# toutane/arcanefem

Hardware: AMD Instinct MI355X
Metric: MDoF/s assembly + CG iter/s, Poisson-3D P1 at 1/2/4/8 MI355X (higher is better)
Workload: dtype f64; 1 GPU; C2 Poisson-3D P1; n=215, dof_total=10077696, nnz_rank0=150048286, parallelism=z-slab x1, RCCL halo + all-reduce in CG

## Files before the change

arcanefem_amd/_capi.py:

```python
from __future__ import annotations

import ctypes
import os

_HERE = os.path.dirname(os.path.abspath(__file__))
LIB_PATH = os.environ.get("AFEM_LIB") or os.path.join(_HERE, "libafem.so")

AFEM_OK = 0
AFEM_MEM_HOST = 0
AFEM_MEM_DEVICE = 1
AFEM_RHS_ADD = 0
AFEM_RHS_SET = 1
AFEM_SOLVER_AUTO = 0
AFEM_SOLVER_PCG = 1
AFEM_SOLVER_DIRECT = 2
AFEM_NEUMANN_VALUE = 0
AFEM_NEUMANN_NORMAL = 1
AFEM_NEUMANN_TRACTION = 2
UNIQUE_ID_BYTES = 128
ERRORS = {1: "ArgumentException", 2: "HipError", 3: "NotImplementedException", 4: "StateError",
          5: "NotFound", 6: "CommError", 7: "LimitExceeded"}


class AfemError(RuntimeError):
# ... 2 lines not shown
        super().__init__(f"{func}: [{ERRORS.get(code, code)}] {msg}")


class MeshInfo(ctypes.Structure):
    _fields_ = [("dim", ctypes.c_int32), ("nb_node_per_cell", ctypes.c_int32), ("n_nodes", ctypes.c_int64),
                ("n_own_nodes", ctypes.c_int64), ("n_cells", ctypes.c_int64)]


class SubdomainInfo(ctypes.Structure):
    _fields_ = [("n_own_nodes", ctypes.c_int64), ("n_nodes", ctypes.c_int64), ("n_cells", ctypes.c_int64),
                ("n_neighbors", ctypes.c_int), ("n_send", ctypes.c_int64), ("n_recv", ctypes.c_int64)]


class CsrView(ctypes.Structure):
    _fields_ = [("n_block_rows", ctypes.c_int64), ("n_block_cols", ctypes.c_int64), ("nnz_blocks", ctypes.c_int64),
                ("block_size", ctypes.c_int32), ("ordered_per_block", ctypes.c_int32), ("rows", ctypes.c_void_p),
                ("columns", ctypes.c_void_p), ("values", ctypes.c_void_p)]


class AssemblyView(ctypes.Structure):
    _fields_ = [("n_rows", ctypes.c_int64), ("n_nodes", ctypes.c_int64), ("n_cells", ctypes.c_int64),
                ("nb_node_per_cell", ctypes.c_int32), ("block_size", ctypes.c_int32),
                ("ordered_per_block", ctypes.c_int32), ("dim", ctypes.c_int32), ("cell_node", ctypes.c_void_p),
                ("coords", ctypes.c_void_p), ("rows", ctypes.c_void_p), ("columns", ctypes.c_void_p),
                ("values", ctypes.c_void_p), ("error_flag", ctypes.c_void_p), ("stream", ctypes.c_void_p)]


class FunctorPlan(ctypes.Structure):
    _fields_ = [("n_units", ctypes.c_int64), ("n_stages", ctypes.c_int64), ("n_entries", ctypes.c_int64),
                ("rows_per_layer", ctypes.c_int32), ("width", ctypes.c_int32), ("nbuf", ctypes.c_int32),
                ("wide", ctypes.c_int32), ("block_size", ctypes.c_int32), ("nb_node_per_cell", ctypes.c_int32),
                ("ordered_per_block", ctypes.c_int32), ("lattice", ctypes.c_int32), ("units", ctypes.c_void_p),
                ("stage_ptr", ctypes.c_void_p), ("layer_rows", ctypes.c_void_p), ("entries", ctypes.c_void_p),
                ("entries2", ctypes.c_void_p), ("rows", ctypes.c_void_p), ("values", ctypes.c_void_p),
                ("stream", ctypes.c_void_p), ("patterns", ctypes.c_void_p), ("n_patterns", ctypes.c_int64),
                ("packed", ctypes.c_int32), ("reserved0", ctypes.c_int32)]


class Csr32View(ctypes.Structure):
    _fields_ = [("n_rows", ctypes.c_int64), ("nnz", ctypes.c_int64), ("rows", ctypes.c_void_p),
                ("rows_nb_column", ctypes.c_void_p), ("columns", ctypes.c_void_p), ("values", ctypes.c_void_p),
                ("identity", ctypes.c_int32)]


class BsrStats(ctypes.Structure):
    _fields_ = [("n_incidences", ctypes.c_int64), ("inc_table_entries", ctypes.c_int64),
                ("max_row_len", ctypes.c_int32), ("rows_per_block", ctypes.c_int32), ("max_seg", ctypes.c_int64),
                ("max_slice_nodes", ctypes.c_int32), ("max_slice_width", ctypes.c_int32),
                ("n_slices", ctypes.c_int64), ("brick_order", ctypes.c_int32), ("uniform_slices", ctypes.c_int32),
                ("last_kernel", ctypes.c_int32), ("stencil_slices", ctypes.c_int32),
                ("stencil_sig", ctypes.c_int32), ("shared_strip_slices", ctypes.c_int64),
                ("uniform_instance_slices", ctypes.c_int64), ("general_slices", ctypes.c_int64),
                ("cube_lattice", ctypes.c_int32), ("cube_axes", ctypes.c_int32),
                ("cube_row_stride", ctypes.c_int64)]


class SolverOpts(ctypes.Structure):
    _fields_ = [("method", ctypes.c_int32), ("max_iter", ctypes.c_int32), ("rtol", ctypes.c_double),
                ("atol", ctypes.c_double), ("check_every", ctypes.c_int32), ("fixed_iterations", ctypes.c_int32),
                ("initial_guess", ctypes.c_int32), ("precond_block", ctypes.c_int32), ("multigrid", ctypes.c_int32),
                ("profile_comm", ctypes.c_int32), ("amg", ctypes.c_int32)]


class SolveStats(ctypes.Structure):
    _fields_ = [("iterations", ctypes.c_int32), ("converged", ctypes.c_int32), ("rel_residual", ctypes.c_double),
                ("residual_norm", ctypes.c_double), ("solve_ms", ctypes.c_double), ("spmv_kernel", ctypes.c_int32),
                ("halo_wait_ms", ctypes.c_double), ("allreduce_ms", ctypes.c_double), ("halo_bytes", ctypes.c_int64),
                ("n_halo", ctypes.c_int32), ("n_allreduce", ctypes.c_int32), ("amg_levels", ctypes.c_int32),
                ("amg_coarse_rows", ctypes.c_int64), ("amg_complexity", ctypes.c_double),
                ("amg_setup_ms", ctypes.c_double), ("precond_ms", ctypes.c_double)]


class StepTiming(ctypes.Structure):
    _fields_ = [("assemble_ms", ctypes.c_double), ("rhs_ms", ctypes.c_double), ("bc_ms", ctypes.c_double),
                ("solve_ms", ctypes.c_double), ("precond_ms", ctypes.c_double), ("update_ms", ctypes.c_double),
                ("total_ms", ctypes.c_double), ("iterations", ctypes.c_int32), ("reserved0", ctypes.c_int32),
                ("nnz_blocks", ctypes.c_int64), ("n_incidences", ctypes.c_int64), ("n_nodes", ctypes.c_int64),
                ("n_own_nodes", ctypes.c_int64)]


ALLREDUCE_FN = ctypes.CFUNCTYPE(ctypes.c_int, ctypes.c_void_p, ctypes.POINTER(ctypes.c_double), ctypes.c_int64)
EXCHANGE_FN = ctypes.CFUNCTYPE(ctypes.c_int, ctypes.c_void_p, ctypes.c_int, ctypes.POINTER(ctypes.c_int32),
                               ctypes.POINTER(ctypes.c_double), ctypes.POINTER(ctypes.c_int64),
                               ctypes.POINTER(ctypes.c_double), ctypes.POINTER(ctypes.c_int64))


class HostTransport(ctypes.Structure):
    _fields_ = [("user", ctypes.c_void_p), ("allreduce_sum", ALLREDUCE_FN), ("exchange", EXCHANGE_FN)]


class NewmarkParams(ctypes.Structure):
    _fields_ = [("E", ctypes.c_double), ("nu", ctypes.c_double), ("rho", ctypes.c_double), ("dt", ctypes.c_double),
                ("body_force", ctypes.c_double * 3), ("penalty", ctypes.c_double), ("gamma", ctypes.c_double),
                ("beta", ctypes.c_double), ("etam", ctypes.c_double), ("etak", ctypes.c_double),
                ("alpm", ctypes.c_double), ("alpf", ctypes.c_double), ("scheme", ctypes.c_int32),
                ("reserved0", ctypes.c_int32)]


P = ctypes.c_void_p
PP = ctypes.POINTER(ctypes.c_void_p)
I32 = ctypes.c_int32
I64 = ctypes.c_int64
U64 = ctypes.c_uint64
D = ctypes.c_double
INT = ctypes.c_int

SIGNATURES = {
# ... 124 lines not shown
```

arcanefem_amd/core.py:

```python
from __future__ import annotations

import ctypes

import numpy as np

from . import _capi as C
from ._capi import AfemError, call

__all__ = ["AfemError", "Context", "Mesh", "BSRFormat", "DoFLinearSystem", "HipDoFLinearSystemFactory",
           "applyNeumannToRhs", "device_count", "set_variant", "structured_halo_plan"]


def _ptr(a: np.ndarray):
    return ctypes.c_void_p(a.ctypes.data)


def _rhs_mode(mode: str) -> int:
    if mode not in ("add", "set"):
        raise ValueError(f"rhs_mode must be 'add' or 'set', got {mode!r}")
    return C.AFEM_RHS_ADD if mode == "add" else C.AFEM_RHS_SET


NEUMANN_MODES = {"value": C.AFEM_NEUMANN_VALUE, "normal": C.AFEM_NEUMANN_NORMAL, "traction": C.AFEM_NEUMANN_TRACTION}

# ... 175 lines not shown
    def __init__(self, mesh: Mesh, nb_dof: int = 1):
        self.mesh = mesh
        self.nb_dof = nb_dof
        self.h = None

    def initialize(self, use_csr_in_linear_system: bool = True):
        h = ctypes.c_void_p()
        call("afem_bsr_create", self.mesh.h, self.nb_dof, 1 if use_csr_in_linear_system else 0, ctypes.byref(h))
        self.h = h
        return self

    def computeSparsity(self):
        call("afem_bsr_compute_sparsity", self.h)

    def assemblePoissonP1(self, coef: float = 1.0, f: float | None = None, rhs_dptr: int | None = None,
                          rhs_mode: str = "add"):
        call("afem_bsr_assemble_poisson_p1_ex", self.h, coef, 0.0 if f is None else f,
             ctypes.c_void_p(rhs_dptr) if rhs_dptr else None, _rhs_mode(rhs_mode))

    def assembleElasticityP1(self, lam: float, mu2: float):
        call("afem_bsr_assemble_elasticity_p1", self.h, lam, mu2)

    def assembleElasticityP1Ex(self, lam: float, mu2: float, mass_coef: float = 0.0, body_force=None,
                               rhs_dptr: int | None = None, rhs_mode: str = "add"):
        f = None
        if body_force is not None:
            f = (ctypes.c_double * 3)(*[float(x) for x in body_force])
        call("afem_bsr_assemble_elasticity_p1_ex", self.h, lam, mu2, mass_coef, f,
             ctypes.c_void_p(rhs_dptr) if rhs_dptr else None, _rhs_mode(rhs_mode))

    def resetMatrixValues(self):
        call("afem_bsr_reset_values", self.h)

    def setValue(self, row: int, col: int, v: float):
        call("afem_bsr_set_value", self.h, row, col, v)

    def getValue(self, row: int, col: int) -> float:
        v = ctypes.c_double()
        call("afem_bsr_get_value", self.h, row, col, ctypes.byref(v))
        return v.value

    def toLinearSystem(self, ls: "DoFLinearSystem"):
        call("afem_bsr_to_linear_system", self.h, ls.impl)

    def view(self) -> C.CsrView:
        v = C.CsrView()
        call("afem_bsr_view", self.h, ctypes.byref(v))
        return v

    def stats(self) -> dict:
        s = C.BsrStats()
        call("afem_bsr_get_stats", self.h, ctypes.byref(s))
        return {k: getattr(s, k) for k, _ in s._fields_}

    def functor_plan(self) -> dict:
        p = C.FunctorPlan()
        call("afem_bsr_functor_plan", self.h, ctypes.byref(p))
        return {k: getattr(p, k) for k, _ in p._fields_ if not k in
                ("units", "stage_ptr", "layer_rows", "entries", "entries2", "rows", "values", "stream",
                 "patterns", "reserved0")}

    def download(self):
        v = self.view()
        rows = np.empty(v.n_block_rows + 1, dtype=np.int64)
        cols = np.empty(v.nnz_blocks, dtype=np.int32)
        vals = np.empty(v.nnz_blocks * v.block_size ** 2, dtype=np.float64)
        call("afem_bsr_download", self.h, _ptr(rows), _ptr(cols), _ptr(vals))
        return rows, cols, vals

    def export_csr32(self):
        n = ctypes.c_int64()
        nnz = ctypes.c_int64()
        call("afem_bsr_get_sizes", self.h, ctypes.byref(n), ctypes.byref(nnz))
        rows = np.empty(n.value, dtype=np.int32)
        rnc = np.empty(n.value, dtype=np.int32)
        cols = np.empty(nnz.value, dtype=np.int32)
        vals = np.empty(nnz.value, dtype=np.float64)
        call("afem_bsr_export_csr32", self.h, _ptr(rows), _ptr(rnc), _ptr(cols), _ptr(vals))
        return rows, rnc, cols, vals

    def close(self):
        if self.h:
            call("afem_bsr_destroy", self.h)
            self.h = None


class DoFLinearSystem:

    def __init__(self):
        self.impl = None
        self.ctx = None
        self.factory = None
        self.n_rows = 0
        self.n_cols = 0

    def setLinearSystemFactory(self, factory: "HipDoFLinearSystemFactory"):
        self.factory = factory

    def initialize(self, ctx: Context, n_rows: int, n_cols_local: int | None = None, solver_name: str = "Solver"):
        factory = self.factory or HipDoFLinearSystemFactory()
        self.impl = factory.createInstance(ctx, n_rows, n_cols_local, solver_name)
        self.ctx = ctx
        self.n_rows = n_rows
        self.n_cols = n_rows if n_cols_local is None else n_cols_local
        return self

# ... 223 lines not shown
```

arcanefem_amd/csrc/afem_internal.hpp:

```cpp
#pragma once

#include <hip/hip_runtime.h>

#include <cstdint>
#include <map>
#include <memory>
#include <stdexcept>
#include <string>
#include <thread>
#include <utility>
#include <vector>

#include "../../include/arcanefem_amd.h"

namespace afem {

#ifndef AFEM_NT_STORES
#define AFEM_NT_STORES 0
#endif
template <class T>
__device__ __forceinline__ void st_out(T* p, T v)
{
#if AFEM_NT_STORES
  __builtin_nontemporal_store(v, p);
// ... 142 lines not shown
  DevBuf<int64_t> inc_slice_ptr;
  DevBuf<int32_t> inc_slice_k;
  int64_t inc_pad_off = 0;
  DevBuf<int32_t> slice_w;
  DevBuf<int64_t> lidx_ptr;
  DevBuf<uint16_t> lidx;
  DevBuf<int64_t> snode_ptr;
  DevBuf<int32_t> snode;
  int max_slice_nodes = 0, max_slice_w = 0, max_slice_k = 0;
  bool strip_ok = false;
  int max_strip_c = 0;
  DevBuf<uint8_t> strip;
  DevBuf<uint8_t> strip_u;
  DevBuf<int64_t> strip_ptr;
  DevBuf<int32_t> strip_c;
  DevBuf<int32_t> strip_n;
  DevBuf<uint8_t> dslot;
  DevBuf<uint64_t> spat;
  DevBuf<uint8_t> uslot;
  DevBuf<SliceRec> rec_u, rec_m, rec_all;
  int64_t n_uni = 0, n_mix = 0;
  DevBuf<SliceRec> rec_ms, rec_mb;
  int64_t n_ms = 0, n_mb = 0;
  int64_t n_msl = 0;
  int msl_nodes = 0;
  int ms_nodes = 0, mb_nodes = 0, mb_w = 0;
  int u_nodes = 0, u_w = 0;
  DevBuf<SliceRec> rec_k, rec_ur;
  DevBuf<uint8_t> urslot;
  DevBuf<SliceRec> rec_k0, rec_u1;
  DevBuf<uint8_t> u1slot;
  int64_t n_k0 = 0, n_u1 = 0;
  int64_t n_k = 0, n_ur = 0;
  int sig_k = -1, k_nodes = 0, ur_nodes = 0, ur_w = 0;
  int64_t n_strip_shared = 0;
  bool rec_ok = false;
  DevBuf<int64_t> pos_rb;
  DevBuf<uint32_t> pos_dl;
  DevBuf<unsigned long long> tickets;
  int64_t ticket_gen = 0;
  int64_t n_slices = 0;
  int64_t n_incidences = 0;
  int max_row_len = 0;
  int64_t max_wave_seg = 0;
  DevBuf<int64_t> diag_pos;
  bool canon = false;
  DevBuf<uint8_t> cperm;
  bool cube_ok = false;
  int64_t cube_L[3] = { 0, 0, 0 };
  bool cube_natural = false;
  int nat_axes[3] = { 0, 1, 2 };
  int64_t nat_L[3] = { 0, 0, 0 };
  int64_t cube_row_stride = 0;
  DevBuf<int32_t> cube_phys;
  DevBuf<int64_t> cube_rb;
  DevBuf<uint64_t> cube_slot;
  DevBuf<int32_t> cube_lat;
  DevBuf<uint64_t> cube_pinv;
};

struct LinearSystem;

struct FunctorPlan {
  bool valid = false;
  int nb_dof = 0;
  int rl = 64, w = 0, nbuf = 1, wide = 0, lattice = 0;
  int fx = 0, fy = 0, zs = 1;
  int64_t n_units = 0, n_stages = 0, n_entries = 0, n_coalesced = 0;
  DevBuf<afem_functor_unit> units;
  DevBuf<int64_t> stage_ptr;
  DevBuf<int32_t> layer_rows;
  DevBuf<uint32_t> ent, ent2;
  int packed = 0;
  int64_t n_patterns = 0;
  DevBuf<uint32_t> patterns;
};
void functor_plan_build(struct Bsr& b);

struct HandOver {
  bool valid = false, identity = false;
  int64_t n_rows = 0, nnz = 0;
  DevBuf<int32_t> rows, rnc, cols;
  DevBuf<int64_t> src;
  DevBuf<double> vals;
};

struct Bsr {
  Mesh* mesh = nullptr;
  int nb_dof = 1;
  bool order_per_block = true;
  bool has_sparsity = false;
  Structure s;
  DevBuf<double> values;
  int last_kernel = 0;
  DevBuf<int64_t> csr_rows;
  DevBuf<int32_t> csr_cols;
  DevBuf<double> csr_vals;
  DevBuf<int32_t> gen_flag;
  FunctorPlan fplan;
  HandOver hand;
  DevBuf<double> cube_stage;
};
void bsr_csr32_mapped_build(Bsr& b, const int32_t* dof_of_host, int64_t n_dof_rows);
double* bsr_csr32_mapped_values(Bsr& b);

struct Comm;
// ... 212 lines not shown
```

arcanefem_amd/csrc/capi.cpp:

```cpp
#include <hip/hip_runtime.h>

#include <algorithm>
#include <cstring>
#include <string>
#include <vector>

#include <rocprofiler-sdk-roctx/roctx.h>

#include "afem_internal.hpp"

using namespace afem;

namespace {
thread_local std::string g_last_error;

int fail(int code, const char* msg)
{
  g_last_error = msg ? msg : "unknown error";
  return code;
}
}

#define API_BEGIN try {
#define API_END                                              \
// ... 609 lines not shown
  if (!b->fplan.valid) functor_plan_build(*b);
  const FunctorPlan& P = b->fplan;
  p->n_units = P.n_units;
  p->n_stages = P.n_stages;
  p->n_entries = P.n_entries;
  p->rows_per_layer = P.rl;
  p->width = P.w;
  p->nbuf = P.nbuf;
  p->wide = P.wide;
  p->block_size = b->nb_dof;
  p->nb_node_per_cell = b->mesh->nv;
  p->ordered_per_block = b->order_per_block ? 1 : 0;
  p->lattice = P.lattice;
  p->units = P.units.p;
  p->stage_ptr = P.stage_ptr.p;
  p->layer_rows = P.layer_rows.p;
  p->entries = P.ent.p;
  p->entries2 = P.wide ? P.ent2.p : nullptr;
  p->rows = b->s.row_ptr.p;
  p->values = b->values.p;
  p->stream = (void*)b->mesh->ctx->stream;
  p->patterns = P.packed ? P.patterns.p : nullptr;
  p->n_patterns = P.n_patterns;
  p->packed = P.packed;
  p->reserved0 = 0;
  API_END
}

int afem_bsr_get_stats(afem_bsr* b, afem_bsr_stats* st)
{
  API_BEGIN
  NOT_NULL(b);
  NOT_NULL(st);
  AFEM_REQUIRE(b->has_sparsity, AFEM_ERR_STATE, "no sparsity");
  st->n_incidences = b->s.n_incidences;
  st->inc_table_entries = (int64_t)b->s.inc.n;
  st->max_row_len = b->s.max_row_len;
  st->rows_per_block = afem::assembly_uses_lds(*b) ? 64 : 0;
  st->max_seg = b->s.max_wave_seg;
  st->max_slice_nodes = b->s.max_slice_nodes;
  st->max_slice_width = b->s.max_slice_w;
  st->n_slices = b->s.n_slices;
  st->brick_order = b->s.lattice ? 2 : b->s.brick_order ? 1 : 0;
  st->cube_lattice = b->s.cube_natural ? 2 : (b->s.canon && b->s.cube_ok) ? 3
                     : (b->mesh->st.valid && b->mesh->st.dim == 3 && !b->s.canon) ? 1 : 0;
  st->uniform_slices = (int32_t)b->s.n_uni;
  st->stencil_slices = (int32_t)b->s.n_k;
  st->stencil_sig = b->s.sig_k;
  st->shared_strip_slices = b->s.n_strip_shared;
  st->uniform_instance_slices = b->s.n_ur;
  st->general_slices = b->s.n_ms + b->s.n_mb;
  st->cube_axes = b->s.cube_natural ? b->s.nat_axes[0] + 3 * b->s.nat_axes[1] + 9 * b->s.nat_axes[2] : 0;
  st->cube_row_stride = b->s.cube_row_stride;
  st->last_kernel = b->last_kernel;
  API_END
}

int afem_bsr_get_sizes(afem_bsr* b, int64_t* n_rows, int64_t* nnz)
{
  API_BEGIN
  NOT_NULL(b);
  AFEM_REQUIRE(b->has_sparsity, AFEM_ERR_STATE, "no sparsity");
  if (n_rows) *n_rows = b->s.n_rows * b->nb_dof;
  if (nnz) *nnz = b->s.nnz * b->nb_dof * b->nb_dof;
  API_END
}

int afem_bsr_download(afem_bsr* b, int64_t* rows, int32_t* cols, double* vals)
{
  API_BEGIN
  NOT_NULL(b);
  AFEM_REQUIRE(b->has_sparsity, AFEM_ERR_STATE, "no sparsity");
  Ctx& ctx = *b->mesh->ctx;
  ctx.set_device();
  if (rows) AFEM_HIP(hipMemcpyAsync(rows, b->s.row_ptr.p, b->s.row_ptr.bytes(), hipMemcpyDeviceToHost, ctx.stream));
  if (cols && b->s.nnz)
    AFEM_HIP(hipMemcpyAsync(cols, b->s.cols.p, (size_t)b->s.nnz * sizeof(int32_t), hipMemcpyDeviceToHost, ctx.stream));
  if (vals && b->values.n)
    AFEM_HIP(hipMemcpyAsync(vals, b->values.p, b->values.bytes(), hipMemcpyDeviceToHost, ctx.stream));
  ctx.sync();
  API_END
}

int afem_bsr_export_csr32(afem_bsr* b, int32_t* rows, int32_t* rows_nb_column, int32_t* columns, double* values)
{
  API_BEGIN
  NOT_NULL(b);
  AFEM_REQUIRE(b->has_sparsity, AFEM_ERR_STATE, "no sparsity");
  const int k = b->nb_dof;
  const int64_t ns = b->s.n_rows * k, nnz = b->s.nnz * k * k;
  AFEM_REQUIRE(nnz < (int64_t)INT32_MAX, AFEM_ERR_LIMIT, "the Int32 CSRFormatView cannot hold more than 2^31-1 values");
  Ctx& ctx = *b->mesh->ctx;
  ctx.set_device();
  std::vector<int64_t> srows(ns + 1);
  if (k == 1) {
    AFEM_HIP(hipMemcpyAsync(srows.data(), b->s.row_ptr.p, srows.size() * 8, hipMemcpyDeviceToHost, ctx.stream));
    if (columns && nnz) AFEM_HIP(hipMemcpyAsync(columns, b->s.cols.p, nnz * 4, hipMemcpyDeviceToHost, ctx.stream));
    if (values && nnz) AFEM_HIP(hipMemcpyAsync(values, b->values.p, nnz * 8, hipMemcpyDeviceToHost, ctx.stream));
  }
  else {
    DevBuf<double> tmp;
    if (b->order_per_block) tmp.alloc(nnz);
    bsr_expand_scalar(*b, tmp.p);
    AFEM_HIP(hipMemcpyAsync(srows.data(), b->csr_rows.p, srows.size() * 8, hipMemcpyDeviceToHost, ctx.stream));
    if (columns && nnz) AFEM_HIP(hipMemcpyAsync(columns, b->csr_cols.p, nnz * 4, hipMemcpyDeviceToHost, ctx.stream));
    if (values && nnz)
// ... 849 lines not shown
```

arcanefem_amd/csrc/cubes.hip:

```cpp
#include "afem_internal.hpp"

#include <algorithm>
#include <limits>

#pragma clang diagnostic ignored "-Wpass-failed"

namespace afem {

namespace {

inline unsigned grid_for(int64_t n, int threads) { return (unsigned)((n + threads - 1) / threads); }

struct P3 {
  double x, y, z;
};
__device__ __forceinline__ P3 psub(P3 a, P3 b) { return P3{ a.x - b.x, a.y - b.y, a.z - b.z }; }
__device__ __forceinline__ P3 pcross(P3 a, P3 b)
{
  return P3{ fma(a.y, b.z, -(a.z * b.y)), fma(a.z, b.x, -(a.x * b.z)), fma(a.x, b.y, -(a.y * b.x)) };
}
__device__ __forceinline__ double pdot(P3 a, P3 b) { return fma(a.z, b.z, fma(a.y, b.y, a.x * b.x)); }
__device__ __forceinline__ double precip(double a)
{
  const double r = __builtin_amdgcn_rcp(a);
  const double e = fma(-a, r, 1.0);
  return fma(r, e, r);
}

struct CubeGeom {
  int npx, npy;
  int nzc;
  int k0, k1;
  int ghost_lo, ghost_hi;
  int n_own_layers;
  int64_t L;
  int tx, ty, zs, ns;
  double s_coef;
  double f_meas;
  int full_flush;
  double acc_init;
  int64_t row_stride;
};

__device__ __forceinline__ bool is_local(const CubeGeom& g, int k)
{
  return (k >= g.k0 && k < g.k1) || (k >= 0 && (k == g.ghost_lo || k == g.ghost_hi));
}
__device__ __forceinline__ int local_layer(const CubeGeom& g, int k)
{
  if (k >= g.k0 && k < g.k1) return k - g.k0;
  if (k == g.ghost_lo) return g.n_own_layers;
  return g.n_own_layers + (g.ghost_lo >= 0 ? 1 : 0);
}

__host__ __device__ constexpr int o_of(int dx, int dy, int dz)
{
  return dz < 0 ? (dy < 0 ? (dx < 0 ? 0 : 1) : (dx < 0 ? 2 : 3))
                : dz == 0 ? (dy < 0 ? (dx < 0 ? 4 : 5) : dy == 0 ? (dx < 0 ? 6 : (dx == 0 ? 7 : 8)) : (dx == 0 ? 9 : 10))
                          : (dy == 0 ? (dx == 0 ? 11 : 12) : (dx == 0 ? 13 : 14));
}
constexpr int kOffX[15] = { -1, 0, -1, 0, -1, 0, -1, 0, 1, 0, 1, 0, 1, 0, 1 };
constexpr int kOffY[15] = { -1, -1, 0, 0, -1, -1, 0, 0, 0, 1, 1, 0, 0, 1, 1 };
constexpr int kOffZ[15] = { -1, -1, -1, -1, 0, 0, 0, 0, 0, 0, 0, 1, 1, 1, 1 };

constexpr int kPerm[6][2] = { { 0, 1 }, { 0, 2 }, { 1, 0 }, { 1, 2 }, { 2, 0 }, { 2, 1 } };
__host__ __device__ constexpr int tet_v(int t, int k)
{
  return k == 0 ? 0 : k == 1 ? (1 << kPerm[t][0]) : k == 2 ? ((1 << kPerm[t][0]) | (1 << kPerm[t][1])) : 7;
}
__host__ __device__ constexpr int cbit(int c, int a) { return (c >> a) & 1; }
__host__ __device__ constexpr int edge_o(int a, int b)
{
  return o_of(cbit(b, 0) - cbit(a, 0), cbit(b, 1) - cbit(a, 1), cbit(b, 2) - cbit(a, 2));
}
__host__ __device__ constexpr bool is_edge(int a, int b)
{
  bool e = false;
  for (int t = 0; t < 6; ++t)
    for (int p = 0; p < 4; ++p)
      for (int q = 0; q < 4; ++q)
        if (tet_v(t, p) == a && tet_v(t, q) == b) e = true;
  return e;
// ... 6 lines not shown
  const uint32_t hi = (uint32_t)__builtin_amdgcn_readlane((int)(uint32_t)((uint64_t)v >> 32), L);
  return (int64_t)(((uint64_t)hi << 32) | lo);
}
__device__ __forceinline__ double lane_f64(double v, int L) { return __longlong_as_double(lane_i64(__double_as_longlong(v), L)); }

constexpr int kRun = 7;
constexpr int kRows = 49;
constexpr int kCol = 9;
constexpr int kAcc = 15;

#ifndef AFEM_CUBES_WAVESYNC
#define AFEM_CUBES_WAVESYNC 1
#endif
__device__ __forceinline__ void wave_lds_order()
{
#if AFEM_CUBES_WAVESYNC
  __builtin_amdgcn_fence(__ATOMIC_ACQ_REL, "wavefront");
  __builtin_amdgcn_wave_barrier();
#else
  __syncthreads();
#endif
}

template <bool NT>
__device__ __forceinline__ void put(double* p, double v)
{
  if constexpr (NT)
    __builtin_nontemporal_store(v, p);
  else
    *p = v;
}

struct CubeCanon {
  const int32_t* phys;
  const int64_t* rb;
  const uint64_t* slot;
  double* stage;
};

constexpr int kCubesBase = 16 | 32 | 64 | 256 | 512 | 1024 | 2048;
constexpr int kCubesV = kCubesBase | 4096;

template <int STRIDE>
constexpr int cube_waves() { return STRIDE == 64 ? 2 : 3; }
template <int STRIDE, bool CARRY, bool XEX, bool YEX, bool CANON, bool HAS_RHS, bool RHS_ADD, int DIAG = kCubesV>
__global__ __launch_bounds__(64) __attribute__((amdgpu_waves_per_eu(cube_waves<STRIDE>(), cube_waves<STRIDE>()))) void k_assemble_cubes(
    CubeGeom g, const int64_t* __restrict__ rows, const double* __restrict__ coords, double* __restrict__ vals,
    double* __restrict__ rhs, CubeCanon cc)
{
  __shared__ __align__(16) double acc[2][kAcc][STRIDE];
  constexpr int NCZ = CARRY ? 1 : 2;
  __shared__ double cz[NCZ][3][kCol * kCol];
  const int lane = threadIdx.x;
  const int64_t n_units = (int64_t)g.tx * g.ty * g.ns;
  const int64_t bid = blockIdx.x;
  const int64_t qq = n_units >> 3, rem = n_units & 7, xc = bid & 7, jj = bid >> 3;
  const int64_t u = xc * qq + (xc < rem ? xc : rem) + jj;
  const int utx = (int)(u % g.tx);
  const int uty = (int)((u / g.tx) % g.ty);
  const int seg = (int)(u / ((int64_t)g.tx * g.ty));
  const int cx0 = kRun * utx, cy0 = kRun * uty;
  const int z0 = g.k0 + seg * g.zs;
  const int z1 = min(z0 + g.zs, g.k1);
  const int zc_first = max(z0 - 1, 0);
  const int zc_last = min(z1 - 1, g.nzc - 1);

  const int ci = lane & 7, cj = lane >> 3;
  const int gx = cx0 - 1 + ci, gy = cy0 - 1 + cj;
  const bool cube_in = gx >= 0 && gy >= 0 && gx + 1 < g.npx && gy + 1 < g.npy;
  auto node_xy = [&](int q, int& nx, int& ny) {
    nx = cx0 - 1 + q % kCol;
    ny = cy0 - 1 + q / kCol;
  };
  double pre[2][3];
  int32_t pid[2] = { 0, 0 };
  auto layer_base = [&](int k) { return (int64_t)__builtin_amdgcn_readfirstlane(local_layer(g, k)) * g.L; };
  int64_t xy_id[2];
#pragma unroll
  for (int h = 0; h < 2; ++h) {
    const int q = min(lane + 64 * h, kCol * kCol - 1);
    int nx, ny;
    node_xy(q, nx, ny);
    nx = min(max(nx, 0), g.npx - 1);
    ny = min(max(ny, 0), g.npy - 1);
    xy_id[h] = nx + (int64_t)g.npx * ny;
  }
  auto clamp_layer = [&](int k) { return is_local(g, k) ? k : g.k0; };
  auto prefetch_ids = [&](int k) {
    if constexpr (CANON) {
      const int32_t* const lp = cc.phys + layer_base(clamp_layer(k));
#pragma unroll
      for (int h = 0; h < 2; ++h) pid[h] = lp[xy_id[h]];
    }
  };
  auto load_layer_to = [&](int k, double (&dst)[2][3]) {
    const double* const lc = CANON ? coords : coords + 3 * layer_base(clamp_layer(k));
#pragma unroll
    for (int h = 0; h < 2; ++h) {
      const int64_t n = CANON ? (int64_t)pid[h] : xy_id[h];
      dst[h][0] = lc[3 * n];
      dst[h][1] = lc[3 * n + 1];
      dst[h][2] = lc[3 * n + 2];
    }
  };
  auto load_layer = [&](int k) { load_layer_to(k, pre); };
  auto store_layer = [&](int buf) {
    buf = NCZ == 1 ? 0 : buf;
#pragma unroll
    for (int h = 0; h < 2; ++h) {
      const int q = min(lane + 64 * h, kCol * kCol - 1);
      cz[buf][0][q] = pre[h][0];
      cz[buf][1][q] = pre[h][1];
      cz[buf][2][q] = pre[h][2];
    }
  };
  constexpr bool DROWS = (DIAG & 256) != 0 && STRIDE == 64;
// ... 566 lines not shown
    ++zc;
  }
  auto layer_step = [&](int zc, auto&& fl) {
    prefetch_rows(zc);
    if constexpr ((DIAG & 16) != 0) next_layer(zc + 2);
    wave_lds_order();
    cubes(zc);
    if constexpr ((DIAG & 16) == 0) next_layer(zc + 2);
    wave_lds_order();
    fl(zc);
    store_layer(zc & 1);
  };
#pragma nounroll
  for (int ph = 0; ph < 2; ++ph) {
    const int zend = ph == 0 ? zf0 : zc_last + 1;
#pragma nounroll
    for (; zc < zend; ++zc) layer_step(zc, flush);
    if constexpr (!CANON) {
      if (ph == 0) {
        if constexpr (RS) {
          if (g.row_stride != 0) {
#pragma nounroll
            for (; zc < zf1; ++zc) {
              pf_r = layer_base(zc) + row_xy;
              if constexpr (RHS_ADD) pf_rhs = rhs[pf_r];
              if constexpr ((DIAG & 16) != 0) next_layer(zc + 2);
              wave_lds_order();
              cubes(zc);
              if constexpr ((DIAG & 16) == 0) next_layer(zc + 2);
              wave_lds_order();
              if constexpr (!(DIAG & 8)) flush_full(zc, run_base);
              store_layer(zc & 1);
#pragma unroll
              for (int q = 0; q < kRun; ++q) run_base[q] += g.row_stride;
            }
          }
        }
#pragma nounroll
        for (; zc < zf1; ++zc)
          layer_step(zc, [&](int z) {
            if constexpr (!(DIAG & 8)) flush_full(z, nullptr);
          });
      }
    }
  }
  if (zc_last + 1 >= z0 && zc_last + 1 < z1) {
    prefetch_rows(zc_last + 1);
    if constexpr (CARRY) {
      add_top(zc_last);
      wave_lds_order();
    }
    flush(zc_last + 1);
  }
}

__global__ void k_cube_stage_maps(int64_t n, int npx, int npy, int nzc, const int32_t* __restrict__ phys,
                                  const uint64_t* __restrict__ slot, int32_t* __restrict__ lat,
                                  uint64_t* __restrict__ pinv)
{
  const int64_t i = (int64_t)blockIdx.x * blockDim.x + threadIdx.x;
  if (i >= n) return;
  const int64_t L = (int64_t)npx * npy;
  const int z = (int)(i / L);
  const int64_t rem = i - (int64_t)z * L;
  const int y = (int)(rem / npx), x = (int)(rem - (int64_t)y * npx);
  uint32_t mask = 0;
  for (int o = 0; o < 15; ++o) {
    const int xx = x + kOffX[o], yy = y + kOffY[o], zz = z + kOffZ[o];
    if (xx >= 0 && yy >= 0 && xx < npx && yy < npy && zz >= 0 && zz <= nzc) mask |= 1u << o;
  }
  const uint64_t sl = slot[i];
  uint64_t w = 0;
  for (int o = 0; o < 15; ++o)
    if ((mask >> o) & 1u) {
      const int t = __popc(mask & ((1u << o) - 1u));
      const int pos = (int)((sl >> (4 * t)) & 15u);
      w |= (uint64_t)o << (4 * pos);
    }
  const int32_t r = phys[i];
  lat[r] = (int32_t)i;
  pinv[r] = w;
}

constexpr int kUnLine = 18;
template <bool HAS_RHS, bool RHS_ADD, int UV = 3>
__global__ __launch_bounds__(64) void k_cube_unstage(int64_t n, const int64_t* __restrict__ rp,
                                                      const int32_t* __restrict__ lat,
                                                      const uint64_t* __restrict__ pinv,
                                                      const double* __restrict__ stage, double f_meas,
                                                      double* __restrict__ vals, double* __restrict__ rhs)
{
  __shared__ __align__(16) double line[64 * kUnLine];
  __shared__ __align__(16) double out[64 * 15 + 2];
  const int lane = threadIdx.x;
  const int64_t r0 = (int64_t)blockIdx.x * 64;
  const int64_t r = r0 + lane;
  const bool valid = r < n;
  const int64_t rc = valid ? r : n - 1;
  const int64_t rb = rp[rc], re = rp[rc + 1];
  const int64_t li = lat[rc];
  const uint64_t m = pinv[rc];
  typedef double d2a __attribute__((ext_vector_type(2), aligned(16)));
  const int part = lane & 7;
  d2a w[8];
#pragma unroll
  for (int k = 0; k < 8; ++k) {
// ... 35 lines not shown
          __builtin_nontemporal_store(d2a{ out[j], out[j + 1] }, reinterpret_cast<d2a*>(g));
        else
          *reinterpret_cast<d2a*>(g) = d2a{ out[j], out[j + 1] };
      }
      else if (lo)
        g[0] = out[j];
      else if (hi)
        g[1] = out[j + 1];
    }
  }
}

__global__ void k_row_stride_check(const int64_t* __restrict__ rows, int64_t L, int64_t l0, int64_t l1, int64_t C,
                                   int32_t* __restrict__ bad)
{
  const int64_t i = (int64_t)blockIdx.x * blockDim.x + threadIdx.x;
  if (i >= (l1 - l0) * L) return;
  const int64_t r = l0 * L + i;
  if (rows[r + L] - rows[r] != C) *bad = 1;
}

bool cube_lattice_geom(const Mesh& m, const Structure& S, int nb_dof, CubeGeom& g, bool& canon)
{
  const StructuredInfo& st = m.st;
  if (m.nv != 4 || nb_dof != 1) return false;
  const bool natural = S.cube_natural;
  canon = !natural && S.canon && S.cube_ok;
  if (!canon && !natural && (!st.valid || st.dim != 3 || S.canon || st.lx > 0 || st.ly > 0 || st.n < 1)) return false;
  if (canon || natural) {
    const int64_t* Lc = natural ? S.nat_L : S.cube_L;
    g.npx = (int)Lc[0];
    g.npy = (int)Lc[1];
    g.nzc = (int)Lc[2] - 1;
    g.k0 = 0;
    g.k1 = (int)Lc[2];
    g.ghost_lo = g.ghost_hi = -1;
    g.L = Lc[0] * Lc[1];
  }
  else {
    g.npx = g.npy = st.n + 1;
    g.nzc = st.nz;
    g.k0 = st.k0;
    g.k1 = st.k1;
    g.ghost_lo = st.ghost_lo;
    g.ghost_hi = st.ghost_hi;
    g.L = st.L;
    if (g.L != (int64_t)g.npx * g.npy) return false;
  }
  g.n_own_layers = g.k1 - g.k0;
  if (g.n_own_layers <= 0 || g.nzc < 1 || g.npx < 2 || g.npy < 2) return false;
  g.tx = (g.npx + kRun - 1) / kRun;
  g.ty = (g.npy + kRun - 1) / kRun;
  return true;
}

}

void cube_row_stride(const Mesh& m, Structure& S, int nb_dof)
{
  S.cube_row_stride = 0;
  CubeGeom g{};
  bool canon = false;
  if (!cube_lattice_geom(m, S, nb_dof, g, canon) || canon) return;
  const int64_t lmax = std::min(g.k1, g.nzc) - g.k0;
  if (lmax < 2 || lmax * g.L > S.n_rows) return;
  Ctx& ctx = *m.ctx;
  int64_t h[2] = { 0, 0 };
  AFEM_HIP(hipMemcpyAsync(&h[0], S.row_ptr.p + g.L, sizeof(int64_t), hipMemcpyDeviceToHost, ctx.stream));
  AFEM_HIP(hipMemcpyAsync(&h[1], S.row_ptr.p + 2 * g.L, sizeof(int64_t), hipMemcpyDeviceToHost, ctx.stream));
  ctx.sync();
  const int64_t C = h[1] - h[0];
  if (C <= 0) return;
  int32_t bad = 0;
  const int64_t n_pairs = (lmax - 2) * g.L;
  if (n_pairs > 0) {
    DevBuf<int32_t> flag;
    flag.alloc(1);
    AFEM_HIP(hipMemsetAsync(flag.p, 0, flag.bytes(), ctx.stream));
    hipLaunchKernelGGL(k_row_stride_check, dim3(grid_for(n_pairs, 256)), dim3(256), 0, ctx.stream, S.row_ptr.p, g.L,
                       (int64_t)1, lmax - 1, C, flag.p);
    AFEM_LAUNCHED();
    AFEM_HIP(hipMemcpyAsync(&bad, flag.p, sizeof(bad), hipMemcpyDeviceToHost, ctx.stream));
    ctx.sync();
  }
  S.cube_row_stride = bad ? 0 : C;
}

bool assemble_cubes(Bsr& b, double coef, double f, double* rhs, int rhs_add)
{
  const Mesh& m = *b.mesh;
  Structure& S = b.s;
  const char* ce = variant("AFEM_ASSEMBLY_CUBES");
  if (ce && atoi(ce) == 0) return false;
  CubeGeom g{};
  bool canon = false;
  if (!cube_lattice_geom(m, S, b.nb_dof, g, canon)) return false;
  Ctx& ctx = *m.ctx;
  g.row_stride = S.cube_row_stride;
  const char* ze = variant("AFEM_CUBES_ZS");
  g.zs = std::max(1, ze ? atoi(ze) : std::min(48, std::max(8, std::max(g.npx, g.npy) / 16)));
  g.ns = (g.n_own_layers + g.zs - 1) / g.zs;
  g.s_coef = coef / 6.0;
  g.f_meas = f / 24.0;
  const char* fe = variant("AFEM_CUBES_FULL");
  g.full_flush = (fe && atoi(fe) == 0) ? 0 : 1;
  const char* ie = variant("AFEM_CUBES_ACC_INIT");
  g.acc_init = (ie && (ie[0] == 'n' || ie[0] == 'N')) ? std::numeric_limits<double>::quiet_NaN() : 0.0;
  const int64_t n_units = (int64_t)g.tx * g.ty * g.ns;
  AFEM_REQUIRE(n_units < (int64_t(1) << 31), AFEM_ERR_LIMIT, "cube kernel: too many units");
  const char* se = variant("AFEM_CUBES_STRIDE");
  const bool s49 = se && atoi(se) == 49;
  const char* ke = variant("AFEM_CUBES_CARRY");
  const bool carry = canon || !(ke && atoi(ke) == 0);
  const char* xe = variant("AFEM_CUBES_XEX");
  const bool xex = canon || (carry && !(xe && atoi(xe) == 0));
  const char* ye = variant("AFEM_CUBES_YEX");
  const bool yex = canon || (xex && !(ye && atoi(ye) == 0));
#define AFEM_CUBES_K(S, C, X, Y, N, D)                                                                               \
  (rhs ? (rhs_add ? &k_assemble_cubes<S, C, X, Y, N, true, true, D> : &k_assemble_cubes<S, C, X, Y, N, true, false, D>) \
       : &k_assemble_cubes<S, C, X, Y, N, false, false, D>)
  const char* de = variant("AFEM_CUBES_V");
  const int diag = de ? atoi(de) : kCubesV;
  constexpr int kB = kCubesBase;
  auto* kern = canon ? AFEM_CUBES_K(64, true, true, true, true, kB & ~1024)
               : carry ? (xex ? (yex ? (s49 ? AFEM_CUBES_K(49, true, true, true, false, kB)
                                            : ((diag & 4096) ? AFEM_CUBES_K(64, true, true, true, false, kB | 4096)
                                                             : AFEM_CUBES_K(64, true, true, true, false, kB)))
                                     : AFEM_CUBES_K(64, true, true, false, false, kB))
                              : AFEM_CUBES_K(64, true, false, false, false, kB))
                       : (s49 ? AFEM_CUBES_K(49, false, false, false, false, kB)
                              : AFEM_CUBES_K(64, false, false, false, false, kB));
#undef AFEM_CUBES_K
  if (diag != (kB | 4096) && diag != kB && carry && xex && yex && rhs && !rhs_add) {
    switch (diag) {
#define AFEM_CUBES_D(D)                                                                                              \
  case D:                                                                                                            \
    kern = canon ? &k_assemble_cubes<64, true, true, true, true, true, false, (D) & ~(1024 | 4096)>                 \
                 : &k_assemble_cubes<64, true, true, true, false, true, false, D>;                                  \
    break;
      AFEM_CUBES_D(0) AFEM_CUBES_D(112) AFEM_CUBES_D(kB | 1) AFEM_CUBES_D(kB | 4)
      AFEM_CUBES_D(kB | 8) AFEM_CUBES_D(kB | 2) AFEM_CUBES_D(kB & ~512) AFEM_CUBES_D(kB & ~1024)
      AFEM_CUBES_D(kB & ~32) AFEM_CUBES_D(kB & ~2048) AFEM_CUBES_D(kB & ~(1024 | 2048))
      AFEM_CUBES_D(kB | 4096 | 1) AFEM_CUBES_D(kB | 4096 | 4) AFEM_CUBES_D(kB | 4096 | 8)
#undef AFEM_CUBES_D
      default: break;
    }
  }
  CubeCanon cc{ canon ? S.cube_phys.p : nullptr, canon ? S.cube_rb.p : nullptr, canon ? S.cube_slot.p : nullptr,
                nullptr };
  const int64_t n_lat = g.L * (int64_t)(g.nzc + 1);
  const bool staged = canon && (diag & 1024) != 0 && n_lat == S.n_rows;
  if (staged) {
    if (S.cube_lat.n != (size_t)n_lat) {
      S.cube_lat.alloc(n_lat);
      S.cube_pinv.alloc(n_lat);
      hipLaunchKernelGGL(k_cube_stage_maps, dim3(grid_for(n_lat, 256)), dim3(256), 0, ctx.stream, n_lat, g.npx, g.npy,
                         g.nzc, S.cube_phys.p, S.cube_slot.p, S.cube_lat.p, S.cube_pinv.p);
      AFEM_LAUNCHED();
    }
    if (b.cube_stage.n != (size_t)(16 * n_lat)) b.cube_stage.alloc(16 * n_lat);
    cc.stage = b.cube_stage.p;
    kern = &k_assemble_cubes<64, true, true, true, true, false, false, kCubesBase | 1024>;
    if (diag != (kCubesBase | 4096) && diag != kCubesBase) {
      switch (diag) {
#define AFEM_CUBES_S(D)                                                                                              \
  case D:                                                                                                            \
    kern = &k_assemble_cubes<64, true, true, true, true, false, false, D>;                                          \
    break;
        AFEM_CUBES_S(kCubesBase | 1024 | 1) AFEM_CUBES_S(kCubesBase | 1024 | 4) AFEM_CUBES_S(kCubesBase & ~2048)
#undef AFEM_CUBES_S
        default: break;
      }
    }
  }
  hipLaunchKernelGGL(kern, dim3((unsigned)n_units), dim3(64), 0, ctx.stream, g, S.row_ptr.p, m.coords.p, b.values.p,
                     rhs, cc);
  AFEM_LAUNCHED();
  if (staged) {
    const int64_t n = S.n_rows;
    auto* un = rhs ? (rhs_add ? &k_cube_unstage<true, true> : &k_cube_unstage<true, false>)
                   : &k_cube_unstage<false, false>;
    const char* uve = variant("AFEM_UNSTAGE_V");
    const int uv = uve ? atoi(uve) : 3;
    if (rhs && !rhs_add && uv == 0) un = &k_cube_unstage<true, false, 0>;
    if (rhs && !rhs_add && uv == 1) un = &k_cube_unstage<true, false, 1>;
    if (rhs && !rhs_add && uv == 2) un = &k_cube_unstage<true, false, 2>;
    hipLaunchKernelGGL(un, dim3((unsigned)grid_for(n, 64)), dim3(64), 0, ctx.stream, n, S.row_ptr.p, S.cube_lat.p,
                       S.cube_pinv.p, b.cube_stage.p, g.f_meas, b.values.p, rhs);
    AFEM_LAUNCHED();
  }
  b.last_kernel = AFEM_KERNEL_CUBES;
  return true;
}

}
```

include/arcanefem_amd.h:

```cpp
#ifndef ARCANEFEM_AMD_H
#define ARCANEFEM_AMD_H

#include <stddef.h>
#include <stdint.h>

#ifdef __cplusplus
extern "C" {
#endif

#define AFEM_OK 0
#define AFEM_ERR_ARG 1
#define AFEM_ERR_HIP 2
#define AFEM_ERR_NOT_IMPL 3
#define AFEM_ERR_STATE 4
#define AFEM_ERR_NOT_FOUND 5
#define AFEM_ERR_COMM 6
#define AFEM_ERR_LIMIT 7

#define AFEM_MEM_HOST 0
#define AFEM_MEM_DEVICE 1

typedef struct afem_ctx afem_ctx;
typedef struct afem_mesh afem_mesh;
typedef struct afem_bsr afem_bsr;
// ... 42 lines not shown
                        int32_t* send_ids, int64_t* recv_counts, int32_t* recv_ids);
int afem_mesh_create_subdomain(afem_ctx* ctx, int dim, int nb_node_per_cell, int64_t n_nodes, int64_t n_cells,
                               const int32_t* cell_node, const double* coords, const int32_t* node_part, int nranks,
                               int rank, afem_mesh** out);
int afem_mesh_get_info(const afem_mesh* mesh, afem_mesh_info* info);
int afem_mesh_download(afem_mesh* mesh, int32_t* cell_node, double* coords, int64_t* local_to_global);
int afem_mesh_structured_bottom_nodes(afem_mesh* mesh, int32_t* ids, int64_t* count);
int afem_mesh_destroy(afem_mesh* mesh);

typedef struct afem_csr_view {
  int64_t n_block_rows;
  int64_t n_block_cols;
  int64_t nnz_blocks;
  int32_t block_size;
  int32_t ordered_per_block;
  const int64_t* rows;
  const int32_t* columns;
  double* values;
} afem_csr_view;

int afem_bsr_create(afem_mesh* mesh, int nb_dof, int use_csr_in_linear_system, afem_bsr** out);
int afem_bsr_compute_sparsity(afem_bsr* bsr);
int afem_bsr_assemble_poisson_p1(afem_bsr* bsr, double coef, double f, double* rhs);
#define AFEM_RHS_ADD 0
#define AFEM_RHS_SET 1
int afem_bsr_assemble_poisson_p1_ex(afem_bsr* bsr, double coef, double f, double* rhs, int rhs_mode);
int afem_bsr_assemble_elasticity_p1(afem_bsr* bsr, double lambda, double mu2);
int afem_bsr_assemble_elasticity_p1_ex(afem_bsr* bsr, double lambda, double mu2, double mass_coef,
                                       const double* body_force, double* rhs, int rhs_mode);
int afem_bsr_reset_values(afem_bsr* bsr);
int afem_bsr_set_value(afem_bsr* bsr, int32_t row, int32_t col, double v);
int afem_bsr_get_value(afem_bsr* bsr, int32_t row, int32_t col, double* v);
int afem_bsr_view(afem_bsr* bsr, afem_csr_view* view);
typedef struct afem_bsr_stats {
  int64_t n_incidences;
  int64_t inc_table_entries;
  int32_t max_row_len;
  int32_t rows_per_block;
  int64_t max_seg;
  int32_t max_slice_nodes;
  int32_t max_slice_width;
  int64_t n_slices;
  int32_t brick_order;
  int32_t uniform_slices;
  int32_t last_kernel;
  int32_t stencil_slices;
  int32_t stencil_sig;
  int64_t shared_strip_slices;
  int64_t uniform_instance_slices;
  int64_t general_slices;
  int32_t cube_lattice;
  int32_t cube_axes;
  int64_t cube_row_stride;
} afem_bsr_stats;
#define AFEM_KERNEL_NONE 0
#define AFEM_KERNEL_STRIP 1
#define AFEM_KERNEL_SLICE_TILE 2
#define AFEM_KERNEL_GLOBAL 3
#define AFEM_KERNEL_ELAST3_STRIP 4
#define AFEM_KERNEL_ELAST3_ITEM 5
#define AFEM_KERNEL_ELAST3_GLOBAL 6
#define AFEM_KERNEL_ELAST2 7
#define AFEM_KERNEL_ELAST3_WG 8
#define AFEM_KERNEL_ELAST3_BIG 9
#define AFEM_KERNEL_CUBES 10
int afem_bsr_get_stats(afem_bsr* bsr, afem_bsr_stats* stats);
int afem_bsr_get_sizes(afem_bsr* bsr, int64_t* n_scalar_rows, int64_t* nnz_scalar);
int afem_bsr_export_csr32(afem_bsr* bsr, int32_t* rows, int32_t* rows_nb_column, int32_t* columns, double* values);
typedef struct afem_assembly_view {
  int64_t n_rows;
  int64_t n_nodes;
  int64_t n_cells;
  int32_t nb_node_per_cell;
  int32_t block_size;
  int32_t ordered_per_block;
  int32_t dim;
  const int32_t* cell_node;
  const double* coords;
  const int64_t* rows;
  const int32_t* columns;
  double* values;
  int32_t* error_flag;
  void* stream;
} afem_assembly_view;
int afem_bsr_assembly_view(afem_bsr* bsr, afem_assembly_view* view);
typedef struct afem_functor_unit {
  int64_t first_stage;
  int32_t n_stages;
  int32_t flags;
} afem_functor_unit;
typedef struct afem_functor_plan {
  int64_t n_units;
  int64_t n_stages;
  int64_t n_entries;
  int32_t rows_per_layer;
  int32_t width;
  int32_t nbuf;
  int32_t wide;
  int32_t block_size;
  int32_t nb_node_per_cell;
  int32_t ordered_per_block;
  int32_t lattice;
  const afem_functor_unit* units;
  const int64_t* stage_ptr;
  const int32_t* layer_rows;
  const uint32_t* entries;
// ... 174 lines not shown
```

Before: 22700 MDoF/s.

## Schedule cube assembly units via cost-balanced per-XCD unit table

Replaces the implicit block-to-unit mapping in the cube assembly kernel with a host-built table of packed unit records. Units get a modelled cost (boundary layers, full and general flushes) and are split across the 8 XCDs by cumulative cost, then sorted by descending cost within each XCD. Records are interleaved so that consecutive block IDs round-robin over the XCDs. The change also allows variable z-segment patterns and exposes scheduling stats. It aims to reduce XCD load imbalance and tail effects, at the cost of one extra per-block table load, padding blocks that exit early, and a cached host-side build.

```diff
diff --git a/arcanefem_amd/_capi.py b/arcanefem_amd/_capi.py
--- a/arcanefem_amd/_capi.py
+++ b/arcanefem_amd/_capi.py
@@ -78,7 +78,10 @@
                 ("stencil_sig", ctypes.c_int32), ("shared_strip_slices", ctypes.c_int64),
                 ("uniform_instance_slices", ctypes.c_int64), ("general_slices", ctypes.c_int64),
                 ("cube_lattice", ctypes.c_int32), ("cube_axes", ctypes.c_int32),
-                ("cube_row_stride", ctypes.c_int64)]
+                ("cube_row_stride", ctypes.c_int64), ("cube_units", ctypes.c_int64),
+                ("cube_unit_records", ctypes.c_int64), ("cube_unit_table", ctypes.c_void_p),
+                ("cube_xcd_cost_spread", ctypes.c_double), ("cube_sched", ctypes.c_int32),
+                ("reserved0", ctypes.c_int32)]
 
 
 class SolverOpts(ctypes.Structure):
diff --git a/arcanefem_amd/core.py b/arcanefem_amd/core.py
--- a/arcanefem_amd/core.py
+++ b/arcanefem_amd/core.py
@@ -251,6 +251,13 @@
         s = C.BsrStats()
         call("afem_bsr_get_stats", self.h, ctypes.byref(s))
         return {k: getattr(s, k) for k, _ in s._fields_}
+
+    def cube_unit_table(self, ctx: "Context") -> np.ndarray:
+        s = self.stats()
+        w = ctx.to_host(s["cube_unit_table"] or 0, 2 * s["cube_unit_records"], np.uint32)
+        w = w.reshape(-1, 2).astype(np.int64)
+        z0 = w[:, 1] & 0xFFFFFF
+        return np.stack([w[:, 0] & 0xFFFF, w[:, 0] >> 16, z0, z0 + (w[:, 1] >> 24)], 1)
 
     def functor_plan(self) -> dict:
         p = C.FunctorPlan()
diff --git a/arcanefem_amd/csrc/afem_internal.hpp b/arcanefem_amd/csrc/afem_internal.hpp
--- a/arcanefem_amd/csrc/afem_internal.hpp
+++ b/arcanefem_amd/csrc/afem_internal.hpp
@@ -218,6 +218,11 @@
   int nat_axes[3] = { 0, 1, 2 };
   int64_t nat_L[3] = { 0, 0, 0 };
   int64_t cube_row_stride = 0;
+  DevBuf<uint32_t> cube_units;
+  int64_t cube_units_n = 0, cube_units_real = 0;
+  int cube_units_sched = 0;
+  double cube_xcd_spread = 0.0;
+  int64_t cube_units_key[12] = { 0, 0, 0, 0, 0, 0, 0, 0, 0, 0, 0, 0 };
   DevBuf<int32_t> cube_phys;
   DevBuf<int64_t> cube_rb;
   DevBuf<uint64_t> cube_slot;
diff --git a/arcanefem_amd/csrc/capi.cpp b/arcanefem_amd/csrc/capi.cpp
--- a/arcanefem_amd/csrc/capi.cpp
+++ b/arcanefem_amd/csrc/capi.cpp
@@ -685,6 +685,12 @@
   st->general_slices = b->s.n_ms + b->s.n_mb;
   st->cube_axes = b->s.cube_natural ? b->s.nat_axes[0] + 3 * b->s.nat_axes[1] + 9 * b->s.nat_axes[2] : 0;
   st->cube_row_stride = b->s.cube_row_stride;
+  st->cube_units = b->s.cube_units_real;
+  st->cube_unit_records = b->s.cube_units_n;
+  st->cube_unit_table = b->s.cube_units.p;
+  st->cube_xcd_cost_spread = b->s.cube_xcd_spread;
+  st->cube_sched = b->s.cube_units_sched;
+  st->reserved0 = 0;
   st->last_kernel = b->last_kernel;
   API_END
 }
diff --git a/arcanefem_amd/csrc/cubes.hip b/arcanefem_amd/csrc/cubes.hip
--- a/arcanefem_amd/csrc/cubes.hip
+++ b/arcanefem_amd/csrc/cubes.hip
@@ -1,7 +1,9 @@
 #include "afem_internal.hpp"
 
 #include <algorithm>
+#include <cstring>
 #include <limits>
+#include <vector>
 
 #pragma clang diagnostic ignored "-Wpass-failed"
 
@@ -27,7 +29,33 @@
   return fma(r, e, r);
 }
 
+struct CubeUnit {
+  int32_t cx, cy, z0, z1;
+};
+constexpr int kUnitMaxColumns = 1 << 16, kUnitMaxLayer = 1 << 24, kUnitMaxLayers = 255;
+
+#ifdef AFEM_WAVE_TIMES
+constexpr unsigned kCubeWtHalf = 16384;
+__device__ unsigned long long afem_cube_wave_t[3 * 2 * kCubeWtHalf];
+extern "C" int afem_debug_cube_wave_times(unsigned long long* out, int n)
+{
+  return (int)hipMemcpyFromSymbol(out, HIP_SYMBOL(afem_cube_wave_t), sizeof(unsigned long long) * (size_t)(3 * n));
+}
+#define AFEM_CWT(i, v)                                                                               \
+  do {                                                                                               \
+    const unsigned b_ = blockIdx.x, back_ = gridDim.x - b_;                                          \
+    if (threadIdx.x == 0 && (b_ < kCubeWtHalf || back_ <= kCubeWtHalf)) {                            \
+      const unsigned s_ = b_ < kCubeWtHalf ? b_ : 2 * kCubeWtHalf - back_;                           \
+      afem_cube_wave_t[3 * s_ + (i)] = (v);                                                          \
+      afem_cube_wave_t[3 * s_ + 2] = b_;                                                             \
+    }                                                                                                \
+  } while (0)
+#else
+#define AFEM_CWT(i, v) (void)0
+#endif
+
 struct CubeGeom {
+  const uint2* units;
   int npx, npy;
   int nzc;
   int k0, k1;
@@ -140,16 +168,11 @@
   constexpr int NCZ = CARRY ? 1 : 2;
   __shared__ double cz[NCZ][3][kCol * kCol];
   const int lane = threadIdx.x;
-  const int64_t n_units = (int64_t)g.tx * g.ty * g.ns;
-  const int64_t bid = blockIdx.x;
-  const int64_t qq = n_units >> 3, rem = n_units & 7, xc = bid & 7, jj = bid >> 3;
-  const int64_t u = xc * qq + (xc < rem ? xc : rem) + jj;
-  const int utx = (int)(u % g.tx);
-  const int uty = (int)((u / g.tx) % g.ty);
-  const int seg = (int)(u / ((int64_t)g.tx * g.ty));
-  const int cx0 = kRun * utx, cy0 = kRun * uty;
-  const int z0 = g.k0 + seg * g.zs;
-  const int z1 = min(z0 + g.zs, g.k1);
+  const uint2 rec = g.units[blockIdx.x];
+  const int z0 = (int)(rec.y & 0xffffffu), z1 = z0 + (int)(rec.y >> 24);
+  if (z0 >= z1) return;
+  AFEM_CWT(0, __builtin_amdgcn_s_memrealtime());
+  const int cx0 = kRun * (int)(rec.x & 0xffffu), cy0 = kRun * (int)(rec.x >> 16);
   const int zc_first = max(z0 - 1, 0);
   const int zc_last = min(z1 - 1, g.nzc - 1);
 
@@ -822,6 +845,7 @@
     }
     flush(zc_last + 1);
   }
+  AFEM_CWT(1, __builtin_amdgcn_s_memrealtime());
 }
 
 __global__ void k_cube_stage_maps(int64_t n, int npx, int npy, int nzc, const int32_t* __restrict__ phys,
@@ -963,6 +987,114 @@
   g.tx = (g.npx + kRun - 1) / kRun;
   g.ty = (g.npy + kRun - 1) / kRun;
   return true;
+}
+
+constexpr double kCostStart = 0.62;
+constexpr double kCostBelow = 0.81;
+constexpr double kCostFull = 1.0;
+constexpr double kCostGeneral = 1.67;
+constexpr double kCostTop = 0.90;
+constexpr int kXcds = 8;
+
+struct CubeUnitWork {
+  int below, full, general, top;
+};
+CubeUnitWork cube_unit_work(const CubeGeom& g, bool canon, const CubeUnit& u)
+{
+  const int cx0 = kRun * u.cx, cy0 = kRun * u.cy;
+  const int zc_first = std::max(u.z0 - 1, 0), zc_last = std::min(u.z1 - 1, g.nzc - 1);
+  const bool xy_full = cx0 >= 1 && cx0 + kRun <= g.npx - 1 && cy0 >= 1 && cy0 + kRun <= g.npy - 1;
+  const int zhi = zc_last + 1;
+  int zf0 = zhi, zf1 = zhi;
+  if (!canon && xy_full && g.full_flush) {
+    zf0 = std::min(std::max(u.z0, g.k0 + 1), zhi);
+    zf1 = std::max(std::min(zhi, g.nzc), zf0);
+  }
+  CubeUnitWork w;
+  w.below = zc_first < u.z0 ? 1 : 0;
+  w.full = zf1 - zf0;
+  w.general = std::max(zhi - u.z0, 0) - w.full;
+  w.top = (zhi >= u.z0 && zhi < u.z1) ? 1 : 0;
+  return w;
+}
+double cube_unit_cost(const CubeGeom& g, bool canon, const CubeUnit& u)
+{
+  const CubeUnitWork w = cube_unit_work(g, canon, u);
+  return kCostStart + kCostBelow * w.below + kCostFull * w.full + kCostGeneral * w.general + kCostTop * w.top;
+}
+
+void build_cube_units(const Mesh& m, Structure& S, const CubeGeom& g, bool canon, int sched, int band_rows,
+                      const std::vector<int>& pat)
+{
+  int64_t pat_key = 0;
+  for (int p : pat) pat_key = pat_key * 256 + p;
+  const int64_t key[12] = { g.npx, g.npy, g.nzc, g.k0, g.k1, pat_key, (int64_t)pat.size(),
+                            band_rows, g.n_own_layers, canon ? 1 : 0, g.full_flush, sched };
+  if (S.cube_units.p && std::equal(key, key + 12, S.cube_units_key)) return;
+  std::vector<int> cuts{ g.k0 };
+  for (size_t i = 0; cuts.back() < g.k1; ++i) cuts.push_back(std::min(cuts.back() + pat[i % pat.size()], g.k1));
+  const int64_t n_col = (int64_t)g.tx * g.ty, n_units = n_col * (int64_t)(cuts.size() - 1);
+  AFEM_REQUIRE(n_units < (int64_t(1) << 31), AFEM_ERR_LIMIT, "cube kernel: too many units");
+  std::vector<CubeUnit> units((size_t)n_units);
+  std::vector<double> cost((size_t)n_units);
+  double total = 0.0;
+  for (int64_t u = 0; u < n_units; ++u) {
+    const int seg = (int)(u / n_col);
+    units[u] = CubeUnit{ (int32_t)(u % g.tx), (int32_t)((u / g.tx) % g.ty), cuts[seg], cuts[seg + 1] };
+    cost[u] = cube_unit_cost(g, canon, units[u]);
+    total += cost[u];
+  }
+  std::vector<int64_t> list[kXcds];
+  if (sched) {
+    double cum = 0.0;
+    for (int64_t u = 0; u < n_units; ++u) {
+      const int x = std::min(kXcds - 1, (int)(kXcds * (cum + 0.5 * cost[u]) / total));
+      list[x].push_back(u);
+      cum += cost[u];
+    }
+    const int64_t band = band_rows > 0 ? (int64_t)band_rows * g.tx : n_units;
+    for (auto& l : list)
+      std::stable_sort(l.begin(), l.end(), [&](int64_t a, int64_t b) {
+        return a / band != b / band ? a / band < b / band : cost[a] > cost[b];
+      });
+  }
+  else {
+    const int64_t qq = n_units / kXcds, rem = n_units % kXcds;
+    for (int x = 0; x < kXcds; ++x) {
+      const int64_t first = x * qq + std::min<int64_t>(x, rem), count = qq + (x < rem ? 1 : 0);
+      for (int64_t j = 0; j < count; ++j) list[x].push_back(first + j);
+    }
+  }
+  size_t longest = 0;
+  double cmax = 0.0, cmin = std::numeric_limits<double>::max();
+  for (const auto& l : list) {
+    longest = std::max(longest, l.size());
+    if (l.empty()) continue;
+    double c = 0.0;
+    for (int64_t u : l) c += cost[u];
+    cmax = std::max(cmax, c);
+    cmin = std::min(cmin, c);
+  }
+  const int64_t n_rec = sched ? (int64_t)kXcds * (int64_t)longest : n_units;
+  AFEM_REQUIRE(n_rec < (int64_t(1) << 31), AFEM_ERR_LIMIT, "cube kernel: too many units");
+  AFEM_REQUIRE(g.tx <= kUnitMaxColumns && g.ty <= kUnitMaxColumns && g.k1 < kUnitMaxLayer,
+               AFEM_ERR_LIMIT, "cube kernel: a unit does not fit its record");
+  auto packed = [](const CubeUnit& u) {
+    return uint2{ (uint32_t)u.cx | (uint32_t)u.cy << 16, (uint32_t)u.z0 | (uint32_t)(u.z1 - u.z0) << 24 };
+  };
+  std::vector<uint2> table((size_t)n_rec, packed(CubeUnit{ 0, 0, g.k0, g.k0 }));
+  for (int x = 0; x < kXcds; ++x)
+    for (size_t j = 0; j < list[x].size(); ++j) table[kXcds * j + x] = packed(units[list[x][j]]);
+  Ctx& ctx = *m.ctx;
+  S.cube_units.alloc(2 * (size_t)n_rec);
+  AFEM_HIP(hipMemcpyAsync(S.cube_units.p, table.data(), sizeof(uint2) * (size_t)n_rec, hipMemcpyHostToDevice,
+                          ctx.stream));
+  ctx.sync();
+  S.cube_units_n = n_rec;
+  S.cube_units_real = n_units;
+  S.cube_units_sched = sched;
+  S.cube_xcd_spread = cmax / cmin;
+  std::copy(key, key + 12, S.cube_units_key);
 }
 
 }
@@ -1009,16 +1141,22 @@
   Ctx& ctx = *m.ctx;
   g.row_stride = S.cube_row_stride;
   const char* ze = variant("AFEM_CUBES_ZS");
-  g.zs = std::max(1, ze ? atoi(ze) : std::min(48, std::max(8, std::max(g.npx, g.npy) / 16)));
-  g.ns = (g.n_own_layers + g.zs - 1) / g.zs;
+  std::vector<int> pat;
+  for (const char* p = ze; p && *p && pat.size() < 7; p = strchr(p, '/') ? strchr(p, '/') + 1 : "")
+    pat.push_back(std::min(kUnitMaxLayers, std::max(1, atoi(p))));
+  if (pat.empty()) pat.push_back(std::min(48, std::max(8, std::max(g.npx, g.npy) / 16)));
+  g.zs = *std::max_element(pat.begin(), pat.end());
+  g.ns = 0;
   g.s_coef = coef / 6.0;
   g.f_meas = f / 24.0;
   const char* fe = variant("AFEM_CUBES_FULL");
   g.full_flush = (fe && atoi(fe) == 0) ? 0 : 1;
   const char* ie = variant("AFEM_CUBES_ACC_INIT");
   g.acc_init = (ie && (ie[0] == 'n' || ie[0] == 'N')) ? std::numeric_limits<double>::quiet_NaN() : 0.0;
-  const int64_t n_units = (int64_t)g.tx * g.ty * g.ns;
-  AFEM_REQUIRE(n_units < (int64_t(1) << 31), AFEM_ERR_LIMIT, "cube kernel: too many units");
+  const char* sce = variant("AFEM_CUBES_SCHED");
+  const char* be = variant("AFEM_CUBES_BAND");
+  build_cube_units(m, S, g, canon, (sce && atoi(sce) == 0) ? 0 : 1, be ? std::max(0, atoi(be)) : 0, pat);
+  g.units = reinterpret_cast<const uint2*>(S.cube_units.p);
   const char* se = variant("AFEM_CUBES_STRIDE");
   const bool s49 = se && atoi(se) == 49;
   const char* ke = variant("AFEM_CUBES_CARRY");
@@ -1084,8 +1222,8 @@
       }
     }
   }
-  hipLaunchKernelGGL(kern, dim3((unsigned)n_units), dim3(64), 0, ctx.stream, g, S.row_ptr.p, m.coords.p, b.values.p,
-                     rhs, cc);
+  hipLaunchKernelGGL(kern, dim3((unsigned)S.cube_units_n), dim3(64), 0, ctx.stream, g, S.row_ptr.p, m.coords.p,
+                     b.values.p, rhs, cc);
   AFEM_LAUNCHED();
   if (staged) {
     const int64_t n = S.n_rows;
diff --git a/include/arcanefem_amd.h b/include/arcanefem_amd.h
--- a/include/arcanefem_amd.h
+++ b/include/arcanefem_amd.h
@@ -118,6 +118,12 @@
   int32_t cube_lattice;
   int32_t cube_axes;
   int64_t cube_row_stride;
+  int64_t cube_units;
+  int64_t cube_unit_records;
+  const uint32_t* cube_unit_table;
+  double cube_xcd_cost_spread;
+  int32_t cube_sched;
+  int32_t reserved0;
 } afem_bsr_stats;
 #define AFEM_KERNEL_NONE 0
 #define AFEM_KERNEL_STRIP 1
```

After: 23450 MDoF/s (median of 6 runs). 1.03x the previous value.
